# pettni/smooth_feedback

Hardware: AMD Instinct MI355X
Metric: QP solves/sec (higher is better)
Workload: dtype f64

## Files before the change

### smooth_feedback_amd/csrc/capi_sparse.hip

```cpp
#include <hip/hip_runtime.h>

#include <algorithm>
#include <chrono>
#include <cstdio>
#include <map>
#include <mutex>
#include <string>
#include <vector>

#include "../../include/sfb.h"
#include "capi_common.h"
#include "qp_sparse_kernel.h"
#include "sparse_plan.h"

struct sfb_sparse_qp_plan {
  sfb::SparsePlanHost host;
  bool pruned = false;
  sfb::SparsePlanHost full;
  std::vector<int32_t> Aorig, Amasked;
  std::mutex mu;
  struct DevCopy {
    int32_t *blob = nullptr, *blob_full = nullptr;
    sfb::SparsePlanDev dev{}, dev_full{};
  };
  std::map<int, DevCopy> per_device;
  struct HostDev {
    std::mutex mu;
    std::pair<char *, size_t> ws{nullptr, 0};
    int64_t batch = -1;
    uint64_t origin = 0;
    hipStream_t stream = nullptr;
    hipEvent_t uploaded = nullptr;
  };
  std::map<int, HostDev> host_dev;
};

namespace sfb {
const SparsePlanHost &plan_host(const sfb_sparse_qp_plan *plan) { return plan->host; }
const SparsePlanHost &plan_io(const sfb_sparse_qp_plan *plan) { return plan->pruned ? plan->full : plan->host; }
}

namespace {

thread_local uint64_t tl_multi_origin = 0;

sfb_status upload_plan(const sfb::SparsePlanHost &h, const std::vector<int32_t> *Aorig, const std::vector<int32_t> *Amasked,
                       int nnzA_io, int32_t **blob_out, sfb::SparsePlanDev &d)
{
  static const std::vector<int32_t> none;
  const std::vector<int32_t> *arrs[] = {&h.Pp, &h.Pi, &h.Pcol, &h.Ap, &h.Aj, &h.Arow, &h.Acp, &h.Aci, &h.Acpos,
                                        &h.Prp, &h.Prj, &h.Prpos, &h.Sp, &h.Sj, &h.Spos, &h.perm, &h.pinv,
                                        &h.Kp, &h.Ki, &h.Kdesc, &h.Lp, &h.Li, &h.Rp, &h.Rk, &h.Rpos, &h.Rlen,
                                        &h.fmap, &h.fidx, &h.bmap, &h.bidx, &h.Kmap, &h.rptr, &h.rtgt, &h.rab, &h.snptr, &h.snR, &h.poff, &h.pmap, &h.fmask, &h.bmask,
                                        &h.f2s, &h.seg, &h.pmapL, &h.rsplit, &h.KmapL, &h.KdescT, &h.KmapT, &h.ztop, &h.ustream, &h.utype, &h.uomap,
                                        &h.ftpos, Aorig ? Aorig : &none, Amasked ? Amasked : &none};
  constexpr int NA = sizeof(arrs) / sizeof(arrs[0]);
  size_t off[NA + 1];
  off[0] = 0;
  for (int a = 0; a < NA; ++a) off[a + 1] = off[a] + ((arrs[a]->size() + 3) / 4) * 4 + 4;
  const size_t self_words = (sizeof(sfb::SparsePlanDev) + 15) / 16 * 4;
  std::vector<int32_t> blob(off[NA] + self_words, 0);
  for (int a = 0; a < NA; ++a) std::copy(arrs[a]->begin(), arrs[a]->end(), blob.begin() + off[a]);
  int32_t *dblob = nullptr;
  hipError_t e = hipMalloc(reinterpret_cast<void **>(&dblob), blob.size() * sizeof(int32_t));
  if (e != hipSuccess) return sfb::hip_fail(e, "hipMalloc(plan)");
  e = hipMemcpy(dblob, blob.data(), blob.size() * sizeof(int32_t), hipMemcpyHostToDevice);
  if (e != hipSuccess) {
    (void)hipFree(dblob);
    return sfb::hip_fail(e, "hipMemcpy(plan)");
  }
  d.n = h.n; d.m = h.m; d.k = h.k; d.nnzP = h.nnzP; d.nnzA = h.nnzA; d.nnzK = h.nnzK; d.nnzL = h.nnzL;
  const int32_t **ptrs[] = {&d.Pp, &d.Pi, &d.Pcol, &d.Ap, &d.Aj, &d.Arow, &d.Acp, &d.Aci, &d.Acpos,
                            &d.Prp, &d.Prj, &d.Prpos, &d.Sp, &d.Sj, &d.Spos, &d.perm, &d.pinv,
                            &d.Kp, &d.Ki, &d.Kdesc, &d.Lp, &d.Li, &d.Rp, &d.Rk, &d.Rpos, &d.Rlen,
                            &d.fmap, &d.fidx, &d.bmap, &d.bidx, &d.Kmap, &d.rptr, &d.rtgt, &d.rab, &d.snptr, &d.snR, &d.poff, &d.pmap, &d.fmask, &d.bmask,
                            &d.f2s, &d.seg, &d.pmapL, &d.rsplit, &d.KmapL, &d.KdescT, &d.KmapT, &d.ztop, &d.ustream, &d.utype, &d.uomap,
                            &d.ftpos, &d.Aorig, &d.Amasked};
  d.funits = h.funits; d.bunits = h.bunits; d.ftail0 = h.ftail0; d.ftail = h.ftail; d.ffull0 = h.ffull0; d.ffull1 = h.ffull1; d.bfull0 = h.bfull0; d.bfull1 = h.bfull1; d.idx_scale = h.idx_scale; d.rsteps = h.rsteps; d.maxcol = h.maxcol; d.nsn = h.nsn; d.lds_doubles = h.lds_doubles; d.nseg = h.nseg; d.nnzKT = h.nnzKT; d.nztop = h.nztop; d.units = h.units; d.nunits = h.nunits;
  for (int a = 0; a < NA; ++a) *ptrs[a] = dblob + off[a];
  d.nnzA_io = nnzA_io;
  d.nmasked = Amasked ? (int)Amasked->size() - 512 : 0;
  if (!Aorig) d.Aorig = d.Amasked = nullptr;
  if ((e = sfb::sparse_device_words(&d.dev_active, &d.dev_busy)) != hipSuccess) {
    (void)hipFree(dblob);
    return sfb::hip_fail(e, "launch bookkeeping of the device");
  }
  d.self = reinterpret_cast<const sfb::SparsePlanDev *>(dblob + off[NA]);
  e      = hipMemcpy(dblob + off[NA], &d, sizeof(d), hipMemcpyHostToDevice);
  if (e != hipSuccess) {
    (void)hipFree(dblob);
    return sfb::hip_fail(e, "hipMemcpy(plan struct)");
  }
  *blob_out = dblob;
  return SFB_OK;
}

sfb_status plan_on_device(sfb_sparse_qp_plan *plan, const sfb_sparse_qp_plan::DevCopy **out)
{
  int devid = 0;
  hipError_t e = hipGetDevice(&devid);
  if (e != hipSuccess) return sfb::hip_fail(e, "hipGetDevice");
  std::lock_guard<std::mutex> lk(plan->mu);
  auto it = plan->per_device.find(devid);
  if (it != plan->per_device.end()) {
    *out = &it->second;
    return SFB_OK;
  }
  sfb_sparse_qp_plan::DevCopy dc;
  sfb_status st;
  if (plan->pruned) {
    st = upload_plan(plan->host, &plan->Aorig, &plan->Amasked, plan->full.nnzA, &dc.blob, dc.dev);
    if (st != SFB_OK) return st;
    st = upload_plan(plan->full, nullptr, nullptr, plan->full.nnzA, &dc.blob_full, dc.dev_full);
    if (st != SFB_OK) {
      (void)hipFree(dc.blob);
      return st;
    }
  } else {
    st = upload_plan(plan->host, nullptr, nullptr, plan->host.nnzA, &dc.blob, dc.dev);
    if (st != SFB_OK) return st;
  }
  auto ins = plan->per_device.emplace(devid, dc);
  *out     = &ins.first->second;
  return SFB_OK;
}

struct WsLayout {
  size_t item_bytes, main_bytes, pool_off, aux_off, total;
};
WsLayout ws_layout(const sfb_sparse_qp_plan *plan, int64_t batch)
{
  const sfb::SparsePlanHost &h = plan->host;
  WsLayout L{};
  L.item_bytes = sfb::qp_sparse_ws_doubles(h.n, h.m, h.nnzL, h.funits, h.bunits, plan->pruned ? h.nnzA : 0) * sizeof(double);
  L.main_bytes = (size_t)batch * L.item_bytes;
  L.pool_off   = L.main_bytes;
  size_t pool  = 0;
  if (plan->pruned) {
    const sfb::SparsePlanHost &f = plan->full;
    pool = (size_t)std::min<int64_t>(batch, sfb::qp_sparse_fallback_slots()) *
           sfb::qp_sparse_ws_doubles(f.n, f.m, f.nnzL, f.funits, f.bunits, 0) * sizeof(double);
  }
  L.aux_off = L.pool_off + pool;
  L.total   = L.aux_off + (sfb::qp_sparse_aux_bytes(batch) + 15) / 16 * 16;
  return L;
}

sfb_status check_sparse_args(const sfb_sparse_qp_plan *plan, const sfb_qp_params *prm, int64_t batch, const void *Px,
                             const void *q, const void *Ax, const void *l, const void *u, const void *wx,
                             const void *wy, const void *x, const void *y, const void *code)
{
  if (!plan) return sfb::fail(SFB_ERR_INVALID_ARG, "plan is NULL");
  if (!prm) return sfb::fail(SFB_ERR_INVALID_ARG, "prm is NULL");
  if (batch < 0) return sfb::fail(SFB_ERR_INVALID_ARG, "batch < 0");
  if (batch > 0 && (!q || !l || !u || !x || !y || !code || (plan->host.nnzP > 0 && !Px) || (sfb::plan_io(plan).nnzA > 0 && !Ax)))
    return sfb::fail(SFB_ERR_INVALID_ARG, "NULL problem / solution pointer");
  if ((wx == nullptr) != (wy == nullptr))
    return sfb::fail(SFB_ERR_INVALID_ARG, "warm_x and warm_y must both be given or both be NULL");
  if (prm->max_iter > 0xFFFFFFFFll) return sfb::fail(SFB_ERR_INVALID_ARG, "max_iter exceeds uint32");
  if (batch > 0x7FFFFFFFll) return sfb::fail(SFB_ERR_UNSUPPORTED, "batch exceeds 2^31-1 per call");
  if ((size_t)std::max(plan->host.lds_doubles, plan->pruned ? plan->full.lds_doubles : 0) * sizeof(double) > 150 * 1024)
// ... 399 lines not shown
```

### smooth_feedback_amd/csrc/qp_sparse.hip

```cpp
#include <hip/hip_runtime.h>

#include <cstdlib>
#include <map>
#include <mutex>

#include <algorithm>
#include <type_traits>
#include <utility>
#include <cfloat>
#include <cmath>

#include "knobs.h"
#include "../../include/sfb.h"
#include "qp_sparse_kernel.h"
#include "wave_util.h"

#ifndef SFB_SWEEP_ASM
#define SFB_SWEEP_ASM 1
#endif
#ifndef SFB_SWEEP_DEPTH
#define SFB_SWEEP_DEPTH 8
#endif

namespace sfb {
// ... 118 lines not shown
  }
}

template<int DEPTH, bool PIPE>
__device__ __forceinline__ void trailing_block(const double *pan, const double *mul, const int R, const int wd,
                                               const int (&tp)[DEPTH], const unsigned (&ab)[DEPTH], double (&v)[DEPTH],
                                               double *ACC)
{
  int ra[DEPTH], rb[DEPTH];
#pragma unroll
  for (int dd = 0; dd < DEPTH; ++dd) {
    ra[dd] = wd + (int)(ab[dd] & 0xFFFFu);
    rb[dd] = wd + (int)(ab[dd] >> 16);
  }
  if constexpr (PIPE) {
    double a[DEPTH], b[DEPTH];
#pragma unroll
    for (int dd = 0; dd < DEPTH; ++dd) {
      a[dd] = pan[ra[dd]];
      b[dd] = mul[rb[dd]];
    }
    for (int jj = 0; jj < wd; ++jj) {
      const int jn = (jj + 1 < wd) ? jj + 1 : jj;
      double an[DEPTH], bn[DEPTH];
#pragma unroll
      for (int dd = 0; dd < DEPTH; ++dd) {
        an[dd] = pan[jn * R + ra[dd]];
        bn[dd] = mul[jn * R + rb[dd]];
      }
#pragma unroll
      for (int dd = 0; dd < DEPTH; ++dd) v[dd] = fma(-a[dd], b[dd], v[dd]);
#pragma unroll
      for (int dd = 0; dd < DEPTH; ++dd) {
        a[dd] = an[dd];
        b[dd] = bn[dd];
      }
    }
  } else {
    for (int jj = 0; jj < wd; ++jj) {
      double a[DEPTH], b[DEPTH];
#pragma unroll
      for (int dd = 0; dd < DEPTH; ++dd) {
        a[dd] = pan[jj * R + ra[dd]];
        b[dd] = mul[jj * R + rb[dd]];
      }
#pragma unroll
      for (int dd = 0; dd < DEPTH; ++dd) v[dd] = fma(-a[dd], b[dd], v[dd]);
    }
  }
#pragma unroll
  for (int dd = 0; dd < DEPTH; ++dd) ACC[tp[dd]] = v[dd];
}

constexpr int kPanelCols = 16;

template<int W>
__device__ __forceinline__ bool panel_eliminate_w(double (&reg)[kPanelCols], const int wd, const int R, double *pan,
                                                  double *mul, const int lane)
{
#pragma unroll
  for (int jj = 0; jj < W; ++jj) {
    if (jj < wd) {
      const double d = lane_bcast(reg[jj], jj);
      if (d == 0.0) return false;
      const double v  = reg[jj] / d;
      const double mv = v * d;
      if (lane > jj) reg[jj] = v;
      if (lane < R) {
        pan[jj * R + lane] = reg[jj];
        mul[jj * R + lane] = mv;
      }
#pragma unroll
      for (int rb = jj + 1; rb < W; ++rb) reg[rb] = fma(-v, lane_bcast(mv, rb), reg[rb]);
    }
  }
  return true;
}
__device__ __forceinline__ bool panel_eliminate(double (&reg)[kPanelCols], const int wd, const int R, double *pan, double *mul,
                                                const int lane)
{
  return panel_eliminate_w<kPanelCols>(reg, wd, R, pan, mul, lane);
}

#ifndef SFB_COPY_DEPTH
#define SFB_COPY_DEPTH 16
#endif
#ifndef SFB_COPY_UB
#define SFB_COPY_UB 8
#endif
template<int DEPTH>
__device__ __forceinline__ void ldl_sweep_copies(const SparsePlanDev &pl, const Ws &w, const int lane)
{
  const int k = uni(pl.k), nnzL = uni(pl.nnzL);
  const double *ACC = w.Lx;
  auto gather_copy = [&](const int32_t *__restrict__ map, double *__restrict__ dst, const int total) {
    int srcn[DEPTH];
#pragma unroll
    for (int dd = 0; dd < DEPTH; ++dd) srcn[dd] = map[lane + dd * kWave];
    for (int q0 = lane; q0 < total; q0 += kWave * DEPTH) {
      int src[DEPTH];
      double v[DEPTH];
#pragma unroll
      for (int dd = 0; dd < DEPTH; ++dd) src[dd] = srcn[dd];
#pragma unroll
      for (int dd = 0; dd < DEPTH; ++dd) v[dd] = ACC[src[dd] >= 0 ? src[dd] : nnzL + k + 1];
      if (q0 + kWave * DEPTH < total) {
#pragma unroll
        for (int dd = 0; dd < DEPTH; ++dd) srcn[dd] = map[q0 + kWave * DEPTH + dd * kWave];
      }
#pragma unroll
      for (int dd = 0; dd < DEPTH; ++dd) __builtin_nontemporal_store(v[dd], &dst[q0 + dd * kWave]);
    }
  };
  static_assert(kSweepPadDev * 2 >= DEPTH, "copy loop assumes whole blocks");
  wave_sync();
  gather_copy(pl.fmap, w.LxF, (uni(pl.funits) + kSweepPadDev) * 2 * kWave);
  gather_copy(pl.bmap, w.LxB, (uni(pl.bunits) + kSweepPadDev) * 2 * kWave);
  wave_sync();
}

typedef int vint4u __attribute__((ext_vector_type(4)));
template<int DEPTH>
__device__ inline int ldl_numeric_units(const SparsePlanDev &pl, const Item &it, const Ws &w, double *t, const int mode,
                                        const double c, const double sigma, const double delta, const int lane,
                                        unsigned long long *fill_ticks = nullptr)
{
  unsigned long long fclk = fill_ticks ? wall_clock64() : 0ull;
  auto fill_lap = [&](const bool is_fill) {
    if (fill_ticks) {
      const unsigned long long now = wall_clock64();
      if (is_fill) *fill_ticks += now - fclk;
      fclk = now;
    }
  };
  const int nnzL = uni(pl.nnzL);
#ifdef SFB_PROF_LDL
  unsigned long long pt[6] = {0, 0, 0, 0, 0, 0}, pc = __builtin_amdgcn_s_memtime();
#define SFB_ULAP(i) { const unsigned long long now_ = __builtin_amdgcn_s_memtime(); pt[i] += now_ - pc; pc = now_; }
#else
#define SFB_ULAP(i)
#endif
  double *ACC = w.Lx;
  for (int z = 0, nz = uni(pl.nztop); z < nz; ++z) {
    const int z0 = uni(pl.ztop[2 * z]), zn = uni(pl.ztop[2 * z + 1]);
    for (int p = lane; p < zn; p += kWave) ACC[z0 + p] = 0.0;
  }
  wave_sync();
  kkt_fill<4>(pl.KdescT, pl.KmapT, 0, uni(pl.nnzKT), it, w, ACC, mode, c, sigma, delta, lane);
  wave_sync();
  SFB_ULAP(0)
  fill_lap(true);
  const vint4u *__restrict__ stream = reinterpret_cast<const vint4u *>(pl.ustream);
  auto at = [&](const unsigned off) -> double & { return *reinterpret_cast<double *>(reinterpret_cast<char *>(t) + off); };
  bool zero_pivot = false;
  constexpr int UB = SFB_COPY_UB;
  for (int sg = 0, nseg = uni(pl.nseg); sg < nseg; ++sg) {
    const int32_t *sgp = pl.seg + 12 * sg;
    const int u0 = uni(sgp[0]), u1 = uni(sgp[1]), c0 = uni(sgp[2]), c1 = uni(sgp[3]), closed = uni(sgp[4]), nLs = uni(sgp[5]);
    const int accN = uni(sgp[6]), kp0 = uni(sgp[7]), kp1 = uni(sgp[8]), gL = uni(sgp[9]), nout = uni(sgp[10]);
    const int32_t *__restrict__ omap = pl.uomap + uni(sgp[11]);
    const int sink = accN + nout;
    if (closed) {
      for (int e = lane; e < accN; e += kWave) t[e] = 0.0;
      wave_lds_fence();
      kkt_fill<4>(pl.Kdesc, pl.KmapL, kp0, kp1, it, w, t, mode, c, sigma, delta, lane);
    } else {
      for (int e0 = lane; e0 < accN; e0 += kWave * UB) {
        double v[UB];
#pragma unroll
        for (int e = 0; e < UB; ++e) {
          const int x = e0 + e * kWave;
          v[e] = (x < accN) ? ACC[x < nLs ? gL + x : nnzL + c0 + (x - nLs)] : 0.0;
        }
#pragma unroll
        for (int e = 0; e < UB; ++e)
          if (e0 + e * kWave < accN) t[e0 + e * kWave] = v[e];
      }
    }
    for (int e0 = lane; e0 < nout; e0 += kWave * UB) {
      int src[UB];
      double v[UB];
#pragma unroll
      for (int e = 0; e < UB; ++e) src[e] = omap[e0 + e * kWave];
#pragma unroll
      for (int e = 0; e < UB; ++e) v[e] = ACC[src[e]];
#pragma unroll
      for (int e = 0; e < UB; ++e)
        if (e0 + e * kWave < nout) t[accN + e0 + e * kWave] = v[e];
    }
    if (lane < 3) t[sink + lane] = (lane == 2) ? 1.0 : 0.0;
    wave_lds_fence();
    SFB_ULAP(1)
    fill_lap(true);
    {
      typedef const __attribute__((address_space(1))) vint4u *gstream_t;
      gstream_t sp = (gstream_t)(stream + (size_t)u0 * kWave + lane);
      auto fetch = [&](vint4u (&q)[DEPTH]) {
#pragma unroll
        for (int d = 0; d < DEPTH; ++d) q[d] = sp[d * kWave];
        sp += DEPTH * kWave;
      };
// ... 214 lines not shown
      tp0[dd] = pl.rtgt[(s0 + dd) * kWave + lane];
      ab0[dd] = (unsigned)pl.rab[(s0 + dd) * kWave + lane];
      if (s0 + dd >= s1) {
        tp0[dd] = pad;
        ab0[dd] = 0u;
      }
    }
#pragma unroll
    for (int dd = 0; dd < DEPTH; ++dd) acc0[dd] = ACC[tp0[dd]];
    const int32_t *pm = pl.pmap + uni(pl.poff[sn]);
    const int npan    = wd * R;
    if (R <= kWave) {
      double reg[kPanelCols];
      int src[kPanelCols];
#pragma unroll
      for (int jj = 0; jj < kPanelCols; ++jj)
        src[jj] = (jj < wd && lane < R) ? pm[jj * R + lane] : pad + 1;
#pragma unroll
      for (int jj = 0; jj < kPanelCols; ++jj) reg[jj] = ACC[src[jj]];
      SFB_LAP(3)
      if (!panel_eliminate(reg, wd, R, pan, mul, lane)) return 0;
#pragma unroll
      for (int jj = 0; jj < kPanelCols; ++jj)
        if (src[jj] < pad) ACC[src[jj]] = reg[jj];
      wave_lds_fence();
    } else {
    for (int q0 = lane; q0 < npan; q0 += kWave * DEPTH) {
      int src[DEPTH];
      double v[DEPTH];
#pragma unroll
      for (int dd = 0; dd < DEPTH; ++dd) src[dd] = pm[q0 + dd * kWave];
#pragma unroll
      for (int dd = 0; dd < DEPTH; ++dd) v[dd] = ACC[src[dd]];
#pragma unroll
      for (int dd = 0; dd < DEPTH; ++dd)
        if (q0 + dd * kWave < npan) pan[q0 + dd * kWave] = v[dd];
    }
    wave_lds_fence();
    SFB_LAP(3)
    for (int jj = 0; jj < wd; ++jj) {
      const double d = pan[jj * R + jj];
      if (d == 0.0) return 0;
      for (int r = jj + 1 + lane; r < R; r += kWave) {
        const double v  = pan[jj * R + r] / d;
        pan[jj * R + r] = v;
        mul[jj * R + r] = v * d;
      }
      wave_lds_fence();
      for (int rb = jj + 1; rb < wd; ++rb)
        for (int ra = rb + lane; ra < R; ra += kWave)
          pan[rb * R + ra] = fma(-pan[jj * R + ra], mul[jj * R + rb], pan[rb * R + ra]);
      wave_lds_fence();
    }
    for (int q = lane; q < npan; q += kWave) {
      const int dst = pm[q];
      if (dst < pad) ACC[dst] = pan[q];
    }
    }
    SFB_LAP(4)
    for (int jj = lane; jj < wd; jj += kWave) w.Dinv[pl.f2s[j0 + jj]] = 1.0 / pan[jj * R + jj];
    trailing_block<DEPTH, false>(pan, mul, R, wd, tp0, ab0, acc0, ACC);
    for (int s = s0 + DEPTH; s < s1; s += DEPTH) {
      int tp[DEPTH];
      unsigned ab[DEPTH];
      double acc[DEPTH];
#pragma unroll
      for (int dd = 0; dd < DEPTH; ++dd) {
        tp[dd] = pl.rtgt[(s + dd) * kWave + lane];
        ab[dd] = (unsigned)pl.rab[(s + dd) * kWave + lane];
        if (s + dd >= s1) {
          tp[dd] = pad;
          ab[dd] = 0u;
        }
      }
#pragma unroll
      for (int dd = 0; dd < DEPTH; ++dd) acc[dd] = ACC[tp[dd]];
      trailing_block<DEPTH, false>(pan, mul, R, wd, tp, ab, acc, ACC);
    }
    SFB_LAP(5)
    wave_sync();
    SFB_LAP(6)
    }
  }
  ldl_sweep_copies<DEPTH>(pl, w, lane);
  SFB_LAP(7)
#ifdef SFB_PROF_LDL
  if (lane == 0 && (blockIdx.x == 0 || blockIdx.x == gridDim.x - 1))
    printf("[ldl block %u mode %d] zero+top fill %llu  lds fill %llu  lds segments: panel-load %llu elim %llu finals+dinv %llu trailing-lds %llu trailing-hbm %llu rest %llu | top: panel-load %llu  panel-elim %llu  trailing %llu  sync %llu  copies %llu  (cycles)\n",
           blockIdx.x, mode, pt[0], pt[1], pt[8], pt[9], pt[10], pt[11], pt[12], pt[2], pt[3], pt[4], pt[5], pt[6], pt[7]);
#endif
  return 1;
}

typedef double vdouble2 __attribute__((ext_vector_type(2)));
typedef int vint2 __attribute__((ext_vector_type(2)));

template<int OFF, bool NT = false>
__device__ __forceinline__ void stream_load(vdouble2 &v, const vdouble2 *p)
{
  static_assert(OFF >= 0 && OFF < 4096, "immediate offset of global_load");
  if constexpr (NT) asm volatile("global_load_dwordx4 %0, %1, off offset:%2 nt" : "=v"(v) : "v"(p), "n"(OFF));
  else asm volatile("global_load_dwordx4 %0, %1, off offset:%2" : "=v"(v) : "v"(p), "n"(OFF));
}
template<int OFF>
__device__ __forceinline__ void stream_load(vint2 &v, const vint2 *p)
{
  static_assert(OFF >= 0 && OFF < 4096, "immediate offset of global_load");
  asm volatile("global_load_dwordx2 %0, %1, off offset:%2" : "=v"(v) : "v"(p), "n"(OFF));
}
typedef int sint8 __attribute__((ext_vector_type(8)));
template<int OFF>
__device__ __forceinline__ void stream_load_masked(vdouble2 &v, const vdouble2 *p, const int shift)
{
  static_assert(OFF >= 0 && OFF < 4096, "immediate offset of global_load");
  asm volatile("s_lshr_b64 exec, -1, %2\n\tglobal_load_dwordx4 %0, %1, off offset:%3 nt\n\ts_mov_b64 exec, -1"
               : "+v"(v)
               : "v"(p), "s"(shift), "n"(OFF)
               : "scc");
}
__device__ __forceinline__ void mask_fetch(sint8 &m, const int32_t *tab, const int byte_off)
{
  asm volatile("s_load_dwordx8 %0, %1, %2" : "=s"(m) : "s"(tab), "s"(byte_off));
}
__device__ __forceinline__ void mask_wait(sint8 &m) { asm volatile("s_waitcnt lgkmcnt(0)" : "+s"(m)); }
template<int N>
__device__ __forceinline__ void stream_wait(vdouble2 &a, vint2 &b)
{
  asm volatile("s_waitcnt vmcnt(%2)" : "+v"(a), "+v"(b) : "n"(N));
}

constexpr int kAgprFree = 0;
template<int DEPTH, bool BYTEOFF, bool LEAN, bool PRE = false, bool NEXT = false, int RES = 0>
__device__ __forceinline__ void sweep_dev(const int32_t *__restrict__ idx, const int units, const double *vals, double *t,
                                 const int lane, const int32_t *__restrict__ mask32, const int full0, const int full1,
                                 vdouble2 (&lx)[DEPTH], vint2 (&ix)[DEPTH], const int32_t *__restrict__ idx_next = nullptr,
                                 const double *vals_next = nullptr, const int32_t *__restrict__ mask_next = nullptr)
{
  static_assert(!(PRE || NEXT) || (!LEAN && DEPTH == 8), "chained sweeps: cacheable form, prefetch distance 8");
  static_assert(DEPTH <= kSweepPadDev && kSweepPadDev % DEPTH == 0, "schedule padding must cover the prefetch distance");
  static_assert(2 * DEPTH <= 62, "vmcnt is a 6-bit counter");
  static_assert(DEPTH == 8, "one scalar load fetches the lane-mask shifts of a block of 8 units");
  constexpr int NVP = DEPTH / 4, NIP = DEPTH / 8;
  const vdouble2 *vp[NVP];
  const vint2 *ip[NIP];
#pragma unroll
  for (int e = 0; e < NVP; ++e) vp[e] = reinterpret_cast<const vdouble2 *>(vals) + lane + e * 4 * kWave;
#pragma unroll
  for (int e = 0; e < NIP; ++e) ip[e] = reinterpret_cast<const vint2 *>(idx) + lane + e * 8 * kWave;
  if constexpr (!PRE) {
#pragma unroll
    for (int d = 0; d < DEPTH; ++d) lx[d] = vdouble2{0.0, 0.0};
  }
  auto issue = [&]<int D, int MODE>(std::integral_constant<int, D>, std::integral_constant<int, MODE>, const sint8 &mk) {
    if constexpr (MODE == 2) stream_load_masked<(D % 4) * kWave * 16>(lx[D], vp[D / 4], mk[D % 8]);
    else stream_load<(D % 4) * kWave * 16, MODE == 1>(lx[D], vp[D / 4]);
    stream_load<(D % 8) * kWave * 8>(ix[D], ip[D / 8]);
  };
  auto for_units = [&]<int... D>(std::integer_sequence<int, D...>, auto &&fn) { (fn(std::integral_constant<int, D>{}), ...); };
  auto advance = [&](const int by) {
#pragma unroll
    for (int e = 0; e < NVP; ++e) vp[e] += by * kWave;
#pragma unroll
    for (int e = 0; e < NIP; ++e) ip[e] += by * kWave;
  };
  sint8 mk;
  {
    const unsigned long long a = reinterpret_cast<unsigned long long>(mask32);
    const unsigned lo = (unsigned)__builtin_amdgcn_readfirstlane((int)(unsigned)a);
    const unsigned hi = (unsigned)__builtin_amdgcn_readfirstlane((int)(unsigned)(a >> 32));
    mask32 = reinterpret_cast<const int32_t *>(((unsigned long long)hi << 32) | lo);
  }
  if constexpr (LEAN) {
    mask_fetch(mk, mask32, 0);
    mask_wait(mk);
    for_units(std::make_integer_sequence<int, DEPTH>{},
              [&]<int D>(std::integral_constant<int, D> dd) { issue(dd, std::integral_constant<int, 2>{}, mk); });
  } else if constexpr (!PRE && RES > 0) {
// ... 155 lines not shown
      at(cur.t0) = fma(-lx[D].x, a0, b0);
      at(cur.t1) = fma(-lx[D].y, a1, b1);
      if constexpr (D == 0 && MASKED) mask_wait(mk);
      issue(dd, msk, mk);
      cur = nxt;
    });
    advance(DEPTH);
  };
  const int r0 = max(0, min(units, full0 - DEPTH)), r1 = max(r0, min(units, full1 - DEPTH));
  int u0 = 0;
  if constexpr (LEAN) {
    for (; u0 < r0; u0 += DEPTH) block(std::integral_constant<int, 2>{}, u0);
    for (; u0 < r1; u0 += DEPTH) block(std::integral_constant<int, 1>{}, u0);
    for (; u0 < units; u0 += DEPTH) block(std::integral_constant<int, 2>{}, u0);
  } else {
    for (; u0 + (NEXT ? DEPTH : 0) < units; u0 += DEPTH) {
      block(std::integral_constant<int, 0>{}, u0);
    }
    if constexpr (NEXT) {
#pragma unroll
      for (int e = 0; e < NVP; ++e) vp[e] = reinterpret_cast<const vdouble2 *>(vals_next) + lane + e * 4 * kWave;
#pragma unroll
      for (int e = 0; e < NIP; ++e) ip[e] = reinterpret_cast<const vint2 *>(idx_next) + lane + e * 8 * kWave;
      block(std::integral_constant<int, 0>{}, u0);
    }
  }
  if constexpr (NEXT) {
    wave_lds_fence();
  } else {
#pragma unroll
    for (int d = 0; d < DEPTH; ++d) stream_wait<0>(lx[d], ix[d]);
    wave_sync();
  }
}

template<int SD>
__device__ inline void ldl_solve_dev(const SparsePlanDev &pl, const Ws &w, double *t, const int lane, const bool lean,
                                     const double *dinv_lds = nullptr)
{
  const double *const Dinv = dinv_lds ? dinv_lds : w.Dinv;
  const int k = uni(pl.k);
  const bool bo = uni(pl.idx_scale) == 8;
  auto sweep = [&](const int32_t *idx, const int units, const double *vals, const int32_t *mask, const int f0, const int f1) {
    if (lean) {
      vdouble2 lx[SFB_SWEEP_DEPTH];
      vint2 ix[SFB_SWEEP_DEPTH];
      if (bo) sweep_dev<SFB_SWEEP_DEPTH, true, true>(idx, units, vals, t, lane, mask, f0, f1, lx, ix);
      else sweep_dev<SFB_SWEEP_DEPTH, false, true>(idx, units, vals, t, lane, mask, f0, f1, lx, ix);
    } else {
      vdouble2 lx[SD];
      vint2 ix[SD];
      if (bo) sweep_dev<SD, true, false>(idx, units, vals, t, lane, mask, f0, f1, lx, ix);
      else sweep_dev<SD, false, false>(idx, units, vals, t, lane, mask, f0, f1, lx, ix);
    }
  };
  sweep(pl.fidx, uni(pl.funits), w.LxF, pl.fmask, uni(pl.ffull0), uni(pl.ffull1));
  for (int j0 = lane; j0 < k; j0 += kWave * 8) {
    double dv[8];
#pragma unroll
    for (int e = 0; e < 8; ++e) dv[e] = (j0 + e * kWave < k) ? Dinv[j0 + e * kWave] : 0.0;
#pragma unroll
    for (int e = 0; e < 8; ++e)
      if (j0 + e * kWave < k) t[j0 + e * kWave] = dv[e] * t[j0 + e * kWave];
  }
  wave_sync();
  sweep(pl.bidx, uni(pl.bunits), w.LxB, pl.bmask, uni(pl.bfull0), uni(pl.bfull1));
}

constexpr int kLatRegRows = 12;
__host__ __device__ constexpr size_t lat_lds_doubles(const int n, const int m)
{
  const size_t lay = (size_t)(((n + m + 2) + 1) & ~1) + n + 2 * (size_t)m + (n + m) + 8 + (2 * kLatRegRows * 64) / 4 + (kLatRegRows * 64) / 8 + 4;
  const size_t rows = (size_t)(((n + m + 2) + 1) & ~1) + kLatRegRows * 64;
  return lay > rows ? lay : rows;
}
#ifndef SFB_LAT_TAIL
#define SFB_LAT_TAIL 48
#endif
constexpr int kLatTail = SFB_LAT_TAIL;
constexpr int kLatTailMax = 48;
static_assert(kLatTail >= 0 && kLatTail <= kLatTailMax && kLatTail % 8 == 0, "the forward sweep ends on a block of 8 units; lanes 0 .. kLatTail");
constexpr int kLatTailReg0 = 256 - 2 * kLatTail;
constexpr int kLatResident = ((kLatTailReg0 - kAgprFree) / 4) & ~7;
__device__ __forceinline__ int lat_tail_units(const SparsePlanDev &pl)
{
  const int ft = uni(pl.ftail);
  return (kLatTail > 0 && uni(pl.idx_scale) == 8 && uni(pl.ftail0) >= 8) ? (ft < kLatTail ? ft : kLatTail) : 0;
}
__device__ __forceinline__ bool lat_resident_ok(const SparsePlanDev &pl, const int treg) { return uni(pl.funits) - treg >= kLatResident + 16; }
__device__ __forceinline__ void lat_resident_load(const double *LxF, const int lane)
{
  asm volatile("" ::: "a255");
  const vdouble2 *p = reinterpret_cast<const vdouble2 *>(LxF) + lane;
  auto for_units = [&]<int... U>(std::integer_sequence<int, U...>, auto &&fn) { (fn(std::integral_constant<int, U>{}), ...); };
  for_units(std::make_integer_sequence<int, kLatResident / 4>{}, [&]<int G>(std::integral_constant<int, G>) {
    const vdouble2 *pg = p + G * 4 * kWave;
    asm volatile("global_load_dwordx4 a[%1:%2], %0, off\n\t"
                 "global_load_dwordx4 a[%3:%4], %0, off offset:1024\n\t"
                 "global_load_dwordx4 a[%5:%6], %0, off offset:2048\n\t"
                 "global_load_dwordx4 a[%7:%8], %0, off offset:3072"
                 :
                 : "v"(pg), "n"(kAgprFree + 16 * G), "n"(kAgprFree + 16 * G + 3), "n"(kAgprFree + 16 * G + 4), "n"(kAgprFree + 16 * G + 7),
                   "n"(kAgprFree + 16 * G + 8), "n"(kAgprFree + 16 * G + 11), "n"(kAgprFree + 16 * G + 12), "n"(kAgprFree + 16 * G + 15)
                 : "memory");
  });
  asm volatile("s_waitcnt vmcnt(0)" ::: "memory");
}
__device__ __forceinline__ unsigned long long lat_tail_load(const SparsePlanDev &pl, const double *LxF, const int lane, const int treg)
{
  asm volatile("" ::: "a255");
  unsigned long long have = 0;
  const int i0 = uni(pl.ftail) - kLatTail;
  const int32_t *pos = pl.ftpos + (lane + i0);
  auto for_steps = [&]<int... S>(std::integer_sequence<int, S...>, auto &&fn) { (fn(std::integral_constant<int, S>{}), ...); };
  for_steps(std::make_integer_sequence<int, kLatTail>{}, [&]<int S>(std::integral_constant<int, S>) {
    const bool on = S >= kLatTail - treg && lane > S && lane <= kLatTail;
    const int q   = on ? pos[(i0 + S) * kWave] : -1;
    const double *pv = LxF + (q >= 0 ? q : 0);
    asm volatile("global_load_dwordx2 a[%1:%2], %0, off" : : "v"(pv), "n"(kLatTailReg0 + 2 * S), "n"(kLatTailReg0 + 2 * S + 1) : "memory");
    if (q >= 0) have |= 1ull << S;
  });
  asm volatile("s_waitcnt vmcnt(0)" ::: "memory");
  return have;
}
__device__ __forceinline__ void ldl_solve_lat(const SparsePlanDev &pl, const Ws &w, double *t, const int lane, const double *Dinv,
                                              vdouble2 (&lx)[8], vint2 (&ix)[8], const bool pre, const bool next, const bool resident = false,
                                              const int treg = 0, const unsigned long long tail_have = 0)
{
  const int k = uni(pl.k);
  const int fu = uni(pl.funits) - treg;
  if (resident) sweep_dev<8, true, false, false, true, kLatResident>(pl.fidx, fu, w.LxF, t, lane, pl.fmask, 0, 0, lx, ix, pl.bidx, w.LxB, pl.bmask);
  else if (pre) sweep_dev<8, true, false, true, true>(pl.fidx, fu, w.LxF, t, lane, pl.fmask, 0, 0, lx, ix, pl.bidx, w.LxB, pl.bmask);
  else sweep_dev<8, true, false, false, true>(pl.fidx, fu, w.LxF, t, lane, pl.fmask, 0, 0, lx, ix, pl.bidx, w.LxB, pl.bmask);
  if constexpr (kLatTail > 0) {
    if (treg > 0) {
      double *const tl = t + (k - 1 - kLatTail) + lane;
      const bool mine = lane >= kLatTail - treg && lane <= kLatTail;
      double tr = mine ? *tl : 0.0;
      auto for_steps = [&]<int... S>(std::integer_sequence<int, S...>, auto &&fn) { (fn(std::integral_constant<int, S>{}), ...); };
      auto block = [&]<int B>(std::integral_constant<int, B>) {
        if (8 * B + 8 > kLatTail - treg) {
          for_steps(std::make_integer_sequence<int, 8>{}, [&]<int E>(std::integral_constant<int, E>) {
            constexpr int S = 8 * B + E;
            int l0, h0;
            asm volatile("v_accvgpr_read_b32 %0, a[%2] ; lat tail (check_sweep_spills.py)\n\tv_accvgpr_read_b32 %1, a[%3]"
                         : "=v"(l0), "=v"(h0)
                         : "n"(kLatTailReg0 + 2 * S), "n"(kLatTailReg0 + 2 * S + 1));
            const double piv = __hiloint2double(__builtin_amdgcn_readlane(__double2hiint(tr), S), __builtin_amdgcn_readlane(__double2loint(tr), S));
            if ((tail_have >> S) & 1) tr = fma(-__hiloint2double(h0, l0), piv, tr);
          });
        }
      };
      for_steps(std::make_integer_sequence<int, kLatTail / 8>{}, block);
      if (mine && lane > kLatTail - treg) *tl = tr;
      wave_lds_fence();
    }
  }
  for (int j0 = lane; j0 < k; j0 += kWave * 8) {
    double dv[8];
#pragma unroll
    for (int e = 0; e < 8; ++e) dv[e] = (j0 + e * kWave < k) ? Dinv[j0 + e * kWave] : 0.0;
#pragma unroll
    for (int e = 0; e < 8; ++e)
      if (j0 + e * kWave < k) t[j0 + e * kWave] = dv[e] * t[j0 + e * kWave];
  }
  wave_lds_fence();
// ... 2061 lines not shown
```

### smooth_feedback_amd/csrc/qp_sparse_kernel.h

```cpp
#pragma once
#include <hip/hip_runtime.h>

#include <cstdint>

#include "qp_dense_kernel.h"

namespace sfb {

#ifndef SFB_KKT_KINDS
#define SFB_KKT_KINDS
enum { K_P = 0, K_A = 1, K_SIGMA = 2, K_RHO = 3 };
#endif

struct SparsePlanDev {
  int n, m, k, nnzP, nnzA, nnzK, nnzL;
  const int32_t *Pp, *Pi, *Pcol, *Ap, *Aj, *Arow;
  const int32_t *Acp, *Aci, *Acpos, *Prp, *Prj, *Prpos, *Sp, *Sj, *Spos;
  const int32_t *perm, *pinv, *Kp, *Ki, *Kdesc, *Lp, *Li, *Rp, *Rk, *Rpos, *Rlen;
  const int32_t *fmap, *fidx, *bmap, *bidx;
  const int32_t *fmask, *bmask;
  int funits, bunits, idx_scale, ffull0, ffull1, bfull0, bfull1;
  int ftail0, ftail;
  const int32_t *ftpos;
  const int32_t *Kmap, *rptr, *rtgt, *rab;
  int rsteps, maxcol;
  const int32_t *snptr, *snR, *poff, *pmap;
  int nsn, lds_doubles;
  const int32_t *f2s, *seg, *pmapL, *rsplit, *KmapL, *KdescT, *KmapT, *ztop;
  int nseg, nnzKT, nztop;
  const int32_t *ustream, *utype, *uomap;
  int units, nunits;
  int nnzA_io, nmasked;
  const int32_t *Aorig, *Amasked;
  int32_t *dev_active;
  const unsigned long long *dev_busy;
  const SparsePlanDev *self;
};

hipError_t sparse_device_words(int32_t **active, const unsigned long long **busy);

constexpr int kSweepPadDev = 16;
#ifdef __HIPCC__
#define SFB_HD __host__ __device__
#else
#define SFB_HD
#endif
SFB_HD inline size_t qp_sparse_factor_doubles(int n, int m, int nnzL, int funits, int bunits)
{
  return (size_t)nnzL + 2 * ((size_t)n + m) + 2 + (size_t)(funits + bunits + 2 * kSweepPadDev) * 128;
}
SFB_HD inline size_t qp_sparse_polish_offset(int n, int m, int nnzL, int funits, int bunits, int nnzA_compact)
{
  const size_t k   = (size_t)n + m;
  const size_t off = qp_sparse_factor_doubles(n, m, nnzL, funits, bunits) + k + 6 * (size_t)n + 11 * (size_t)m + 16 +
                     (((size_t)nnzA_compact + 1) & ~(size_t)1);
  return (off + 1) & ~(size_t)1;
}
inline size_t qp_sparse_ws_doubles(int n, int m, int nnzL, int funits, int bunits, int nnzA_compact = 0)
{
  const size_t tot = qp_sparse_polish_offset(n, m, nnzL, funits, bunits, nnzA_compact) +
                     qp_sparse_factor_doubles(n, m, nnzL, funits, bunits) + m + 4;
  return (tot + 1) & ~(size_t)1;
}

inline size_t qp_sparse_ws_doubles(const SparsePlanDev &pl)
{
  return qp_sparse_ws_doubles(pl.n, pl.m, pl.nnzL, pl.funits, pl.bunits, pl.Aorig ? pl.nnzA : 0);
}

hipError_t qp_sparse_launch(const SparsePlanDev &pl, const DenseKernelParams &kp, int64_t batch, const double *Px,
                            const double *q, const double *Ax, const double *l, const double *u, const double *wx,
                            const double *wy, double *x, double *y, double *obj, uint32_t *iter, int32_t *code,
                            double *workspace, hipStream_t stream, const int32_t *order = nullptr, int32_t *aux = nullptr,
                            const SparsePlanDev *fallback = nullptr, double *fallback_ws = nullptr,
                            double *trace = nullptr, int trace_cap = 0, double *phase_us = nullptr);
size_t qp_sparse_aux_bytes(int64_t batch);
int qp_sparse_fallback_slots();

}
```

### smooth_feedback_amd/csrc/sparse_plan.cpp

```cpp
#include "knobs.h"
#include "sparse_plan.h"

#include <algorithm>
#include <cstdio>
#include <cstdlib>
#include <iterator>
#include <array>
#include <numeric>
#include <tuple>

namespace sfb {

namespace {

void transpose_pattern(int nouter, int ninner, const std::vector<int32_t> &outer_ptr,
                       const std::vector<int32_t> &inner, std::vector<int32_t> &tp, std::vector<int32_t> &ti,
                       std::vector<int32_t> &tpos)
{
  const int nnz = outer_ptr[nouter];
  tp.assign(ninner + 1, 0);
  ti.resize(nnz);
  tpos.resize(nnz);
  for (int p = 0; p < nnz; ++p) tp[inner[p] + 1]++;
  for (int i = 0; i < ninner; ++i) tp[i + 1] += tp[i];
// ... 886 lines not shown
          std::push_heap(heap.begin(), heap.end());
        }
      }
      return slots;
    };
    Steps slots = schedule(k);
    tail0 = ntail = 0;
    if (forward && o.idx_scale == 8) {
      const int today = (((int)slots.size() + 7) / 8) * 8;
      int best = today + 1, bestT = 0;
      Steps body_best;
      for (int T = 8; T <= SparsePlanHost::kSweepTailMax && T <= k - 1; T += 8) {
        Steps body = schedule(k - 1 - T);
        const int total = (((int)body.size() + 7) / 8) * 8 + T;
        if (total <= best) { best = total; bestT = T; body_best = std::move(body); }
      }
      if (bestT > 0 && best <= today) {
        slots = std::move(body_best);
        slots.resize(((slots.size() + 7) / 8) * 8);
        tail0 = (int)slots.size();
        ntail = bestT;
        for (int j = k - 1 - bestT; j < k - 1; ++j) {
          slots.emplace_back();
          for (int q = col_first[j]; q < col_first[j + 1]; ++q) slots.back().push_back({sl[q].pos, sl[q].tgt, sl[q].piv});
        }
      }
    }
    const int steps = (int)slots.size();
    if (const char *dbg = sfb::knob("SFB_PLAN_DEBUG"); dbg && dbg[0] == '1') {
      fprintf(stderr, "[sfb plan] %s sweep: %d units, slots per unit:", forward ? "forward" : "backward", steps);
      for (int s = 0; s < steps; ++s) fprintf(stderr, " %d", (int)slots[s].size());
      fprintf(stderr, "\n");
    }
    units           = steps;
    units = ((units + 7) / 8) * 8;
    const size_t total = (size_t)(units + SparsePlanHost::kSweepPad) * 128;
    xmap.assign(total, -1);
    const int sc = o.idx_scale;
    xidx.assign(total, (k * sc) | ((k * sc) << 16));
    xmask.assign((size_t)units + 2 * SparsePlanHost::kSweepPad, 63);
    constexpr bool bank_aware = true;
    long cyc_before = 0, cyc_after = 0;
    UnitPlacer up;
    const int search_passes = ns <= 20000 ? 1 : 0;
    for (int s = 0; s < steps; ++s) {
      const int lanes = std::max(1, ((int)slots[s].size() + 1) / 2);
      xmask[s]        = 64 - lanes;
      up.lanes = lanes;
      up.sl.clear();
      for (const auto &e : slots[s]) up.sl.push_back({e[1], e[2]});
      const auto cyc = up.place(search_passes);
      cyc_before += cyc.first;
      cyc_after += bank_aware ? cyc.second : cyc.first;
      for (size_t e = 0; e < slots[s].size(); ++e) {
        const int pos  = bank_aware ? up.where[e] : (int)((e % (size_t)lanes) * 2 + e / (size_t)lanes);
        const size_t q = (size_t)s * 128 + (size_t)pos;
        xmap[q] = acc_of(slots[s][e][0]);
        xidx[q] = (slots[s][e][1] * sc) | ((slots[s][e][2] * sc) << 16);
      }
    }
    if (const char *dbg = sfb::knob("SFB_PLAN_DEBUG"); dbg && dbg[0] == '1')
      fprintf(stderr, "[sfb plan] %s sweep: modelled LDS cycles of the slot accesses per sweep: natural placement %ld, bank-aware %ld (floor %d)\n",
              forward ? "forward" : "backward", cyc_before, cyc_after, 16 * steps);
    full0 = full1 = 0;
    for (int s = 0; s < steps;) {
      if ((int)slots[s].size() != cap) { ++s; continue; }
      int e = s;
      while (e < steps && (int)slots[e].size() == cap) ++e;
      const int a = ((s + 7) / 8) * 8, b = (e / 8) * 8;
      if (b - a > full1 - full0) { full0 = a; full1 = b; }
      s = e;
    }
  };
  build(true, o.fmap, o.fidx, o.funits, o.fmask, o.ffull0, o.ffull1, o.ftail0, o.ftail);
  o.ftpos.assign((size_t)o.ftail * 64, -1);
  for (int i = 0; i < o.ftail; ++i)
    for (int s = 0; s < 128; ++s) {
      const size_t q = (size_t)(o.ftail0 + i) * 128 + s;
      if (o.fmap[q] >= 0) o.ftpos[(size_t)i * 64 + (((uint32_t)o.fidx[q] & 0xFFFFu) / o.idx_scale - (k - 1 - o.ftail))] = (int32_t)q;
    }
  int none0 = 0, none1 = 0;
  build(false, o.bmap, o.bidx, o.bunits, o.bmask, o.bfull0, o.bfull1, none0, none1);

  return true;
}

}
```

### smooth_feedback_amd/csrc/sparse_plan.h

```cpp
#pragma once
#include <cstdint>
#include <vector>

namespace sfb {

#ifndef SFB_KKT_KINDS
#define SFB_KKT_KINDS
enum { K_P = 0, K_A = 1, K_SIGMA = 2, K_RHO = 3 };
#endif

struct SparsePlanHost {
  int n = 0, m = 0, k = 0, nnzP = 0, nnzA = 0, nnzK = 0, nnzL = 0;
  std::vector<int32_t> Pp, Pi, Pcol;
  std::vector<int32_t> Ap, Aj, Arow;
  std::vector<int32_t> Acp, Aci, Acpos;
  std::vector<int32_t> Prp, Prj, Prpos;
  std::vector<int32_t> Sp, Sj, Spos;
  std::vector<int32_t> perm, pinv;
  std::vector<int32_t> Kp, Ki, Kkind, Kidx;
  std::vector<int32_t> Lp, Li;
  std::vector<int32_t> Rp, Rk, Rpos;
  std::vector<int32_t> Rlen;
  static constexpr int kSweepPad = 16;
  std::vector<int32_t> fmap, fidx, bmap, bidx, fmask, bmask;
  int funits = 0, bunits = 0, idx_scale = 1, ffull0 = 0, ffull1 = 0, bfull0 = 0, bfull1 = 0;
  static constexpr int kSweepTailMax = 48;
  int ftail0 = 0, ftail = 0;
  std::vector<int32_t> ftpos;
  std::vector<int32_t> Kmap, rptr, rtgt, rab, snptr, snR, poff, pmap;
  std::vector<int32_t> Kdesc;
  int rsteps = 0, maxcol = 0, nsn = 0, lds_doubles = 0;
  std::vector<int32_t> f2s;
  static constexpr int kSegStride = 12;
  std::vector<int32_t> seg, pmapL, rsplit, KmapL, KdescT, KmapT, ztop;
  int nseg = 0, nnzKT = 0, nztop = 0;
  std::vector<int32_t> ustream, utype, uomap;
  int units = 0, nunits = 0;
};

bool build_sparse_plan(int n, int m, const int32_t *Pp, const int32_t *Pi, const int32_t *Ap, const int32_t *Aj,
                       int ordering, const int32_t *user_perm, const int32_t *stage, SparsePlanHost &out,
                       const char **msg, int lds_hint = 0);

}
```

Measured before the change: 232,700.

## Compact sweep copy lists to skip masked lanes in LDL gather copies

The planner now builds compact forward and backward copy lists. Each entry holds a destination pair index and two source indices, and lanes the sweep masks out are dropped, except for head units and full-block ranges, which keep every lane. The kernel walks these lists and does paired gathers with vectorized nontemporal double2 stores, instead of copying every padded slot of fmap/bmap. This cuts gather and store traffic for empty lanes. In exchange each entry carries a 12-byte index record, the copy depth is halved, and correctness depends on the kernel never reading lanes that are no longer written.

```diff
diff --git a/smooth_feedback_amd/csrc/capi_sparse.hip b/smooth_feedback_amd/csrc/capi_sparse.hip
--- a/smooth_feedback_amd/csrc/capi_sparse.hip
+++ b/smooth_feedback_amd/csrc/capi_sparse.hip
@@ -47,13 +47,15 @@
 sfb_status upload_plan(const sfb::SparsePlanHost &h, const std::vector<int32_t> *Aorig, const std::vector<int32_t> *Amasked,
                        int nnzA_io, int32_t **blob_out, sfb::SparsePlanDev &d)
 {
+  static_assert(sfb::kCopyBlockDev == sfb::SparsePlanHost::kCopyBlock && sfb::kCopyAllLanesUnits == sfb::SparsePlanHost::kCopyAllLanesUnits,
+                "copy lists: planner and kernel agree");
   static const std::vector<int32_t> none;
   const std::vector<int32_t> *arrs[] = {&h.Pp, &h.Pi, &h.Pcol, &h.Ap, &h.Aj, &h.Arow, &h.Acp, &h.Aci, &h.Acpos,
                                         &h.Prp, &h.Prj, &h.Prpos, &h.Sp, &h.Sj, &h.Spos, &h.perm, &h.pinv,
                                         &h.Kp, &h.Ki, &h.Kdesc, &h.Lp, &h.Li, &h.Rp, &h.Rk, &h.Rpos, &h.Rlen,
                                         &h.fmap, &h.fidx, &h.bmap, &h.bidx, &h.Kmap, &h.rptr, &h.rtgt, &h.rab, &h.snptr, &h.snR, &h.poff, &h.pmap, &h.fmask, &h.bmask,
                                         &h.f2s, &h.seg, &h.pmapL, &h.rsplit, &h.KmapL, &h.KdescT, &h.KmapT, &h.ztop, &h.ustream, &h.utype, &h.uomap,
-                                        &h.ftpos, Aorig ? Aorig : &none, Amasked ? Amasked : &none};
+                                        &h.ftpos, &h.fcopy, &h.bcopy, Aorig ? Aorig : &none, Amasked ? Amasked : &none};
   constexpr int NA = sizeof(arrs) / sizeof(arrs[0]);
   size_t off[NA + 1];
   off[0] = 0;
@@ -75,8 +77,8 @@
                             &d.Kp, &d.Ki, &d.Kdesc, &d.Lp, &d.Li, &d.Rp, &d.Rk, &d.Rpos, &d.Rlen,
                             &d.fmap, &d.fidx, &d.bmap, &d.bidx, &d.Kmap, &d.rptr, &d.rtgt, &d.rab, &d.snptr, &d.snR, &d.poff, &d.pmap, &d.fmask, &d.bmask,
                             &d.f2s, &d.seg, &d.pmapL, &d.rsplit, &d.KmapL, &d.KdescT, &d.KmapT, &d.ztop, &d.ustream, &d.utype, &d.uomap,
-                            &d.ftpos, &d.Aorig, &d.Amasked};
-  d.funits = h.funits; d.bunits = h.bunits; d.ftail0 = h.ftail0; d.ftail = h.ftail; d.ffull0 = h.ffull0; d.ffull1 = h.ffull1; d.bfull0 = h.bfull0; d.bfull1 = h.bfull1; d.idx_scale = h.idx_scale; d.rsteps = h.rsteps; d.maxcol = h.maxcol; d.nsn = h.nsn; d.lds_doubles = h.lds_doubles; d.nseg = h.nseg; d.nnzKT = h.nnzKT; d.nztop = h.nztop; d.units = h.units; d.nunits = h.nunits;
+                            &d.ftpos, &d.fcopy, &d.bcopy, &d.Aorig, &d.Amasked};
+  d.funits = h.funits; d.bunits = h.bunits; d.ftail0 = h.ftail0; d.ftail = h.ftail; d.ffull0 = h.ffull0; d.ffull1 = h.ffull1; d.bfull0 = h.bfull0; d.bfull1 = h.bfull1; d.idx_scale = h.idx_scale; d.rsteps = h.rsteps; d.maxcol = h.maxcol; d.nsn = h.nsn; d.lds_doubles = h.lds_doubles; d.nseg = h.nseg; d.nnzKT = h.nnzKT; d.nztop = h.nztop; d.units = h.units; d.nunits = h.nunits; d.fcopy_n = h.fcopy_n; d.bcopy_n = h.bcopy_n;
   for (int a = 0; a < NA; ++a) *ptrs[a] = dblob + off[a];
   d.nnzA_io = nnzA_io;
   d.nmasked = Amasked ? (int)Amasked->size() - 512 : 0;
diff --git a/smooth_feedback_amd/csrc/qp_sparse.hip b/smooth_feedback_amd/csrc/qp_sparse.hip
--- a/smooth_feedback_amd/csrc/qp_sparse.hip
+++ b/smooth_feedback_amd/csrc/qp_sparse.hip
@@ -224,17 +224,57 @@
   return panel_eliminate_w<kPanelCols>(reg, wd, R, pan, mul, lane);
 }
 
+#ifndef SFB_COPY_COMPACT
+#define SFB_COPY_COMPACT 1
+#endif
 #ifndef SFB_COPY_DEPTH
-#define SFB_COPY_DEPTH 16
+#define SFB_COPY_DEPTH (SFB_COPY_COMPACT ? 8 : 16)
 #endif
 #ifndef SFB_COPY_UB
 #define SFB_COPY_UB 8
 #endif
+typedef double vdouble2 __attribute__((ext_vector_type(2)));
+struct CopyEntry { int32_t dst, s0, s1; };
 template<int DEPTH>
 __device__ __forceinline__ void ldl_sweep_copies(const SparsePlanDev &pl, const Ws &w, const int lane)
 {
   const int k = uni(pl.k), nnzL = uni(pl.nnzL);
   const double *ACC = w.Lx;
+#if SFB_COPY_COMPACT
+  static_assert(kCopyBlockDev % (DEPTH * kWave) == 0, "copy loop assumes whole blocks");
+  const int zero = nnzL + k + 1;
+  typedef const __attribute__((address_space(1))) CopyEntry *glist_t;
+  auto fetch = [](glist_t p, const int dd) { return CopyEntry{p[dd * kWave].dst, p[dd * kWave].s0, p[dd * kWave].s1}; };
+  auto gather_copy = [&](const int32_t *list, double *__restrict__ dst, const int total) {
+    glist_t ent = (glist_t)reinterpret_cast<const CopyEntry *>(list) + lane;
+    vdouble2 *out = reinterpret_cast<vdouble2 *>(dst);
+    CopyEntry en[DEPTH];
+#pragma unroll
+    for (int dd = 0; dd < DEPTH; ++dd) en[dd] = fetch(ent, dd);
+    for (int b0 = 0; b0 < total; b0 += kWave * DEPTH) {
+      CopyEntry e[DEPTH];
+      vdouble2 v[DEPTH];
+#pragma unroll
+      for (int dd = 0; dd < DEPTH; ++dd) e[dd] = en[dd];
+#pragma unroll
+      for (int dd = 0; dd < DEPTH; ++dd) {
+        v[dd].x = ACC[e[dd].s0 >= 0 ? e[dd].s0 : zero];
+        v[dd].y = ACC[e[dd].s1 >= 0 ? e[dd].s1 : zero];
+      }
+      if (b0 + kWave * DEPTH < total) {
+        ent += kWave * DEPTH;
+#pragma unroll
+        for (int dd = 0; dd < DEPTH; ++dd) en[dd] = fetch(ent, dd);
+      }
+#pragma unroll
+      for (int dd = 0; dd < DEPTH; ++dd) __builtin_nontemporal_store(v[dd], &out[e[dd].dst]);
+    }
+  };
+  wave_sync();
+  gather_copy(pl.fcopy, w.LxF, uni(pl.fcopy_n));
+  gather_copy(pl.bcopy, w.LxB, uni(pl.bcopy_n));
+  wave_sync();
+#else
   auto gather_copy = [&](const int32_t *__restrict__ map, double *__restrict__ dst, const int total) {
     int srcn[DEPTH];
 #pragma unroll
@@ -259,6 +299,7 @@
   gather_copy(pl.fmap, w.LxF, (uni(pl.funits) + kSweepPadDev) * 2 * kWave);
   gather_copy(pl.bmap, w.LxB, (uni(pl.bunits) + kSweepPadDev) * 2 * kWave);
   wave_sync();
+#endif
 }
 
 typedef int vint4u __attribute__((ext_vector_type(4)));
@@ -639,7 +680,7 @@
     SFB_LAP(6)
     }
   }
-  ldl_sweep_copies<DEPTH>(pl, w, lane);
+  ldl_sweep_copies<SFB_COPY_COMPACT ? SFB_COPY_DEPTH : DEPTH>(pl, w, lane);
   SFB_LAP(7)
 #ifdef SFB_PROF_LDL
   if (lane == 0 && (blockIdx.x == 0 || blockIdx.x == gridDim.x - 1))
@@ -649,7 +690,6 @@
   return 1;
 }
 
-typedef double vdouble2 __attribute__((ext_vector_type(2)));
 typedef int vint2 __attribute__((ext_vector_type(2)));
 
 template<int OFF, bool NT = false>
@@ -971,6 +1011,7 @@
 static_assert(kLatTail >= 0 && kLatTail <= kLatTailMax && kLatTail % 8 == 0, "the forward sweep ends on a block of 8 units; lanes 0 .. kLatTail");
 constexpr int kLatTailReg0 = 256 - 2 * kLatTail;
 constexpr int kLatResident = ((kLatTailReg0 - kAgprFree) / 4) & ~7;
+static_assert(kLatResident <= kCopyAllLanesUnits, "lat_resident_load fetches whole units unmasked: the copy list writes every lane of them");
 __device__ __forceinline__ int lat_tail_units(const SparsePlanDev &pl)
 {
   const int ft = uni(pl.ftail);
diff --git a/smooth_feedback_amd/csrc/qp_sparse_kernel.h b/smooth_feedback_amd/csrc/qp_sparse_kernel.h
--- a/smooth_feedback_amd/csrc/qp_sparse_kernel.h
+++ b/smooth_feedback_amd/csrc/qp_sparse_kernel.h
@@ -35,11 +35,15 @@
   int32_t *dev_active;
   const unsigned long long *dev_busy;
   const SparsePlanDev *self;
+  const int32_t *fcopy, *bcopy;
+  int fcopy_n, bcopy_n;
 };
 
 hipError_t sparse_device_words(int32_t **active, const unsigned long long **busy);
 
 constexpr int kSweepPadDev = 16;
+constexpr int kCopyBlockDev = 512;
+constexpr int kCopyAllLanesUnits = 64;
 #ifdef __HIPCC__
 #define SFB_HD __host__ __device__
 #else
diff --git a/smooth_feedback_amd/csrc/sparse_plan.cpp b/smooth_feedback_amd/csrc/sparse_plan.cpp
--- a/smooth_feedback_amd/csrc/sparse_plan.cpp
+++ b/smooth_feedback_amd/csrc/sparse_plan.cpp
@@ -992,6 +992,25 @@
   int none0 = 0, none1 = 0;
   build(false, o.bmap, o.bidx, o.bunits, o.bmask, o.bfull0, o.bfull1, none0, none1);
 
+  auto copy_list = [&](const bool forward, const std::vector<int32_t> &xmap, const std::vector<int32_t> &xmask, const int units,
+                       const int full0, const int full1, std::vector<int32_t> &list, int &len, int &padded) {
+    const int all = units + SparsePlanHost::kSweepPad;
+    const int head = forward ? std::min(units, (int)SparsePlanHost::kCopyAllLanesUnits) : 0;
+    list.clear();
+    for (int u = 0; u < all; ++u) {
+      const int lanes = (u < head || (u >= full0 && u < full1)) ? 64 : 64 - xmask[u];
+      for (int l = 0; l < lanes; ++l) {
+        const size_t q = ((size_t)u * 64 + l) * 2;
+        list.insert(list.end(), {(int32_t)(u * 64 + l), xmap[q], xmap[q + 1]});
+      }
+    }
+    len    = (int)(list.size() / 3);
+    padded = ((len + SparsePlanHost::kCopyBlock - 1) / SparsePlanHost::kCopyBlock) * SparsePlanHost::kCopyBlock;
+    for (int e = len; e < padded; ++e) list.insert(list.end(), {(int32_t)((all - 1) * 64), -1, -1});
+  };
+  copy_list(true, o.fmap, o.fmask, o.funits, o.ffull0, o.ffull1, o.fcopy, o.fcopy_len, o.fcopy_n);
+  copy_list(false, o.bmap, o.bmask, o.bunits, o.bfull0, o.bfull1, o.bcopy, o.bcopy_len, o.bcopy_n);
+
   return true;
 }
 
diff --git a/smooth_feedback_amd/csrc/sparse_plan.h b/smooth_feedback_amd/csrc/sparse_plan.h
--- a/smooth_feedback_amd/csrc/sparse_plan.h
+++ b/smooth_feedback_amd/csrc/sparse_plan.h
@@ -27,6 +27,10 @@
   static constexpr int kSweepTailMax = 48;
   int ftail0 = 0, ftail = 0;
   std::vector<int32_t> ftpos;
+  static constexpr int kCopyAllLanesUnits = 64;
+  static constexpr int kCopyBlock = 512;
+  std::vector<int32_t> fcopy, bcopy;
+  int fcopy_len = 0, fcopy_n = 0, bcopy_len = 0, bcopy_n = 0;
   std::vector<int32_t> Kmap, rptr, rtgt, rab, snptr, snR, poff, pmap;
   std::vector<int32_t> Kdesc;
   int rsteps = 0, maxcol = 0, nsn = 0, lds_doubles = 0;
```

After: 234,700, median of 6. No clear change (+0.8%).
